# Agzs/BlockMaze

Measured on AMD Instinct MI355X. Metric: Groth16 proofs/sec (send circuit, alt_bn128), higher is better.
Workload: dtype u32 limbs (254-bit Fq/Fr Montgomery; all MSM accumulations, the H query's weighted bucket sum and the transforms' tiles on nine 29-bit limbs)

## Files before the change

### blockmaze_amd/csrc/capi_engine.cpp

```cpp
#include <cstring>
#include <memory>
#include <mutex>
#include <string>
#include <vector>
#include "../../include/zkgpu.h"
#include "gpu.hpp"

namespace zk {
void probe_field(int field, int op, const uint8_t *a, const uint8_t *b, uint8_t *out, size_t n);
void probe_fq2(int op, const uint8_t *a, const uint8_t *b, uint8_t *out, size_t n);
void probe_group(int group, int op, const uint8_t *a, const uint8_t *b, uint8_t *out, size_t n);
}
using namespace zk;
using namespace zk::host;

static thread_local std::string g_err;
void zkgpu_set_error(const std::string &s) { g_err = s; }
std::mutex g_gpu_mutex;

template <class Fn> static int guarded(Fn fn) {
  try { if (!gpu_available()) { g_err = "no HIP device visible; libzkgpu has no CPU fallback"; return ZKGPU_ERR_NO_DEVICE; }
        std::lock_guard<std::mutex> lk(g_gpu_mutex); return fn(); }
  catch (const std::exception &e) { g_err = e.what(); return ZKGPU_ERR_RUNTIME; }
  catch (...) { g_err = "unknown error"; return ZKGPU_ERR_RUNTIME; }
// ... 92 lines not shown
  while (rs < small) rs <<= 1;
  size_t m = (small == rs) ? min_size : big + rs;
  return lg <= 28 ? m : 0;
}
int zkgpu_domain_transform(size_t min_size, int op, uint8_t *data) { return guarded([&] { Domain d(min_size); size_t m = d.m(); DevBuf<Fe32> buf(m);
    buf.upload((const Fe32 *)data, m); fr_to_mont_dev(buf.get(), m);
  switch (op) {
    case 0: d.fft(buf.get(), 1, m);
    break;
    case 1: d.ifft(buf.get(), 1, m);
    break;
    case 2: d.coset_fft(buf.get(), 1, m);
    break;
    case 3: d.icoset_fft(buf.get(), 1, m);
    break;
    default: g_err = "op";
    return ZKGPU_ERR_ARG;
  }
  fr_from_mont_dev(buf.get(), m); buf.download((Fe32 *)data, m); return ZKGPU_OK; }); }

struct zkgpu_r1cs { R1csHost host; std::unique_ptr<R1csDev> dev; std::unique_ptr<Domain> dom; };
zkgpu_r1cs *zkgpu_r1cs_create(size_t n_inputs, size_t n_vars, size_t n_cons, const uint32_t *const rowptr[3], const uint32_t *const col[3],
    const uint8_t *const coeff[3]) {
  zkgpu_r1cs *out = nullptr;
  guarded([&] { std::unique_ptr<zkgpu_r1cs> h(new zkgpu_r1cs); h->host.n_inputs = n_inputs; h->host.n_vars = n_vars; h->host.n_cons = n_cons;
    for (int m = 0; m < 3; m++) {
      size_t nnz = rowptr[m][n_cons];
      h->host.rowptr[m].assign(rowptr[m], rowptr[m] + n_cons + 1);
      h->host.col[m].assign(col[m], col[m] + nnz);
      h->host.coeff[m].resize(nnz);
// ... 21 lines not shown
```

### blockmaze_amd/csrc/gen_field29.py

```python
#!/usr/bin/env python3
Q = 21888242871839275222246405745257275088696311157297823662689037894645226208583
B = 29; M = (1 << B) - 1; NL = 9; RP = 1 << (B * NL)
def limbs29(x, n=NL): return [(x >> (B * i)) & M for i in range(n - 1)] + [x >> (B * (n - 1))]
def adjusted(c):
    l = limbs29(c * Q); lo = 3 * (1 << B) + 64
    for i in range(NL - 1):
        n = 3 if l[i] + 3 * (1 << B) >= lo else 4
        l[i] += n << B; l[i + 1] -= n
        assert lo <= l[i] < 4 << B, (c, i, l[i])
    assert l[NL - 1] > 0 and sum(v << (B * i) for i, v in enumerate(l)) == c * Q
    return l
def adjusted_light(c):
    l = limbs29(c * Q); lo = (1 << B) + 64
    for i in range(NL - 1):
        n = 1 if l[i] + (1 << B) >= lo else 2
        l[i] += n << B; l[i + 1] -= n
        assert lo <= l[i] < lo + (1 << B), (c, i, l[i])
    assert l[NL - 1] > 0 and sum(v << (B * i) for i, v in enumerate(l)) == c * Q
    return l
INV = (-pow(Q, -1, 1 << B)) % (1 << B)
P29 = limbs29(Q); ONE29 = limbs29(RP % Q); RCONV = limbs29((1 << 256) % Q)
KS = {c: adjusted(c) for c in (2, 4, 6, 12, 18)}

RATIO = RP / Q
# ... 304 lines not shown
        for i in range(8): f[i + 1] += f[i] >> B; f[i] &= M
        assert (V % Q == 0) == any(f == limbs29(k * Q) for k in range(5))
lin_check()
BOUNDS_G2 = check_bounds_g2()
prm = ["// GENERATED by gen_field29.py - do not edit.  Constants of Fq on nine 29-bit limbs, for host and device code (verify_sched.hpp).", "#pragma once", "#include <cstdint>", "namespace zk { namespace p29 {"]
def carr(name, v, comment=""): prm.append("constexpr uint32_t %s[9] = {%s};%s" % (name, ", ".join("0x%xu" % x for x in v), ("   // " + comment) if comment else ""))
prm.append("constexpr uint32_t MASK = 0x%xu, INV = 0x%xu, MU = 0x%xu, MU_SHIFT = %d, LIN_MAX_UNITS = %d;   // MU = floor(2^53 / ((p >> 232) + 1)); a linear combination's value stays below LIN_MAX_UNITS p" % (M, INV, MU, MU_SHIFT, LIN_MAX_UNITS))
carr("P", P29, "p"); carr("K6", KS[6], "6 p, low limbs in [3 * 2^29 + 64, 4 * 2^29): K6 - x has no negative limb for x below 6 p with limbs below 3 * (2^29 + 8)"); carr("NP", NP, "2^264 - p (top limb: 32 bits)")
prm.append("constexpr uint32_t KP[5][9] = {%s};   // k p, k = 0 .. 4, exact limbs" % ", ".join("{" + ", ".join("0x%xu" % x for x in limbs29(k * Q)) + "}" for k in range(5)))
prm.append("} }")
open(__file__.replace("gen_field29.py", "field29_params.h"), "w").write("\n".join(prm) + "\n")
EMIT_BARRETT = True; FQ_LINES = gen_struct(); EMIT_BARRETT = False
R_MOD = 21888242871839275222246405745257275088548364400416034343698204186575808495617
Q_SAVE = Q; KS_SAVE = KS; Q = R_MOD; INV = (-pow(Q, -1, 1 << B)) % (1 << B); P29 = limbs29(Q); ONE29 = limbs29(RP % Q); RCONV = limbs29((1 << 256) % Q); KS = {}
FR_LINES = [l.replace("Fq29", "Fr29") for l in gen_struct()]; self_check()
open(__file__.replace("gen_field29.py", "field29_gfx950.inc"), "w").write("\n".join(HEADER + FQ_LINES + FR_LINES) + "\n")
print("bounds:", BOUNDS); print("bounds of the oct addition:", BOUNDS_OCT)
```

### blockmaze_amd/csrc/gpu.hip

```cpp
#include <hip/hip_runtime.h>
#include <cstdio>
#include <cstdlib>
#include <chrono>
#include <cstring>
#include <map>
#include <vector>
#include <algorithm>
#include <mutex>
#include <atomic>
#include <mutex>
#include "gpu_internal.hpp"
#include "ntt.cuh"
#include "ecntt.cuh"

__attribute__((constructor(101))) static void zkgpu_load_time_environment() { setenv("GPU_MAX_HW_QUEUES", "16", 0); }

namespace zk {

constexpr int MAX_LANES_PER_DEVICE = 31, MAX_LANES = 1 + 8 * 28;
static uint8_t g_lane_claimed[MAX_LANES];
static std::atomic<GpuContext *> g_lanes[MAX_LANES];
static std::atomic<int> g_lane_slot[MAX_LANES];
static std::mutex g_lane_mutex;
static thread_local int t_lane = 0;
// ... 227 lines not shown
  if (bytes % 16 || (reinterpret_cast<uintptr_t>(dst) | reinterpret_cast<uintptr_t>(src)) % 16) { HIP_CHECK(hipMemcpyAsync(dst, src, bytes, hipMemcpyDeviceToDevice, gpu().stream)); return; }
  const size_t n16 = bytes / 16; hipLaunchKernelGGL(k_copy_words16, dim3((unsigned)std::min<size_t>(cdiv(n16, 256), 4096)), dim3(256), 0, gpu().stream, (const uint4 *)src, (uint4 *)dst, n16);
}


static size_t ceil_log2(size_t n) { size_t r = ((n & (n - 1)) == 0 ? 0 : 1); while (n > 1) { n >>= 1; r++; } return r; }
using host::HFr;
static HFr fr_root_of_unity(size_t n) {
  HFr w;
  memcpy(w.l, FR_ROOT_OF_UNITY_2_28, 32);
  for (size_t i = 28; i > ceil_log2(n); --i) w = w.sqr();
  return w;
}
static HFr fr_coset_gen() { HFr g; memcpy(g.l, FR_COSET_GEN, 32); return g; }

struct Radix2Tables {
  int logn; size_t n; DevBuf<Fe32> tw, itw, tw261, itw261;
  Radix2Tables(size_t n_, const HFr &w) : logn((int)ceil_log2(n_)), n(n_), tw(n_ / 2 ? n_ / 2 : 1), itw(n_ / 2 ? n_ / 2 : 1), tw261(n_ / 2 ? n_ / 2 : 1),
      itw261(n_ / 2 ? n_ / 2 : 1) {
    std::vector<Fe32> a(n / 2 ? n / 2 : 1), b(a.size()), a5(a.size()), b5(a.size()); HFr wi = w.inv(), x = HFr::one(), y = HFr::one();
    auto times32 = [](HFr v) {
      for (int i = 0; i < 5; i++) v = v + v;
      return v;
    };
    for (size_t j = 0; j < std::max<size_t>(n / 2, 1); j++) {
      memcpy(&a[j], x.l, 32);
      memcpy(&b[j], y.l, 32);
      HFr x5 = times32(x), y5 = times32(y);
      memcpy(&a5[j], x5.l, 32);
      memcpy(&b5[j], y5.l, 32);
      x = x * w;
      y = y * wi;
    }
    tw.upload(a.data(), a.size()); itw.upload(b.data(), b.size()); tw261.upload(a5.data(), a5.size()); itw261.upload(b5.data(), b5.size());
  }
};
static std::vector<Fe32> geometric_table(size_t n, const HFr &first, const HFr &ratio) {
  std::vector<Fe32> t(n);
  HFr x = first;
  for (size_t i = 0; i < n; i++) {
    memcpy(&t[i], x.l, 32);
    x = x * ratio;
  }
  return t;
}

static int ntt_pref_log_c() {
  static const int v = [] {
    const char *e = getenv("ZK_NTT_LOGC");
    int x = e ? atoi(e) : 1;
    return x < 0 ? 0 : x > 3 ? 3 : x; }(); return v; }
static Fe32 fe261(HFr v) {
  for (int i = 0; i < 5; i++) v = v + v;
  Fe32 o;
  memcpy(&o, v.l, 32);
  return o;
}
struct NttCall { Fe32 *data, *scratch; const Fe32 *tw, *tw261; int logn; const Fe32 *pre_scale, *pre261; Fe32 scale261; const Fe32 *post_scale;
    size_t stride, scratch_stride; const Fe32 *out261 = nullptr; };
static int ntt_prio_bits() { static const int v = (int)(zk_prio_bits(ZKP_NTT) >> 24) << 8; return v; }
static int ntt_radix_log() {
  static const int rl = [] {
    const char *e = getenv("ZK_NTT_RADIX_LOG");
    int x = e ? atoi(e) : 2;
    return x < 1 ? 1 : x > 3 ? 3 : x;
  }();
  return rl;
}
static bool ntt_two_pass(int logn) { return logn > NTT_TILE_LOG && logn <= 2 * NTT_TILE_LOG; }
static unsigned ntt_threads_for(int logN, int logC) {
  int g = logN + logC - ntt_radix_log();
  return 1u << (g < 6 ? 6 : g > 8 ? 8 : g);
}
static size_t ntt_lds_for(int logN, int logC) {
  size_t e = (size_t)1 << (logN + logC);
  return sizeof(Fr29) * (e + (e >> 4) + 1) + (sizeof(Fr29) << logN) / 2;
}
static void ntt_raise_lds() {
  static std::atomic<uint64_t> cols_done{0}, rows_done{0};
  zk_raise_dynamic_lds((const void *)k_ntt_cols, 128 * 1024, cols_done); zk_raise_dynamic_lds((const void *)k_ntt_rows, 128 * 1024, rows_done);
}
static void ntt_two_pass_launch(const NttCall *calls, int n_calls, int batch) {
  hipStream_t s = gpu().stream;
  ntt_raise_lds();
  NttJob cj[2], rj[2];
  memset(cj, 0, sizeof cj);
  memset(rj, 0, sizeof rj);
  unsigned tc = 64, tr = 64;
  size_t lc = 0, lr = 0;
  for (int k = 0; k < n_calls; k++) {
    const NttCall &c = calls[k];
    const int l1 = c.logn / 2, l2 = c.logn - l1, c1 = std::min(ntt_pref_log_c(), std::min(NTT_TILE_LOG - l1, l2)), c2 = std::min(ntt_pref_log_c(),
        std::min(NTT_TILE_LOG - l2, l1));
    Fr sc; memcpy(&sc, &c.scale261, 32);
    cj[k] = NttJob{(const Fr *)c.data, (Fr *)c.scratch, (const Fr *)c.pre261, (const Fr *)c.tw261, sc, c.logn, l1, c1, 1u << (l2 - c1), c.stride,
        c.scratch_stride, nullptr};
    rj[k] = NttJob{(const Fr *)c.scratch, (Fr *)c.data, (const Fr *)c.post_scale, (const Fr *)c.tw261, sc, c.logn, l1, c2, 1u << (l1 - c2), c.scratch_stride,
        c.stride, (const Fr *)c.out261};
    tc = std::max(tc, ntt_threads_for(l1, c1));
    tr = std::max(tr, ntt_threads_for(l2, c2));
    lc = std::max(lc, ntt_lds_for(l1, c1));
    lr = std::max(lr, ntt_lds_for(l2, c2));
  }
  hipLaunchKernelGGL(k_ntt_cols, dim3(cj[0].tiles + cj[1].tiles, batch), dim3(tc), lc, s, cj[0], cj[1], ntt_radix_log() | ntt_prio_bits());
  hipLaunchKernelGGL(k_ntt_rows, dim3(rj[0].tiles + rj[1].tiles, batch), dim3(tr), lr, s, rj[0], rj[1], ntt_radix_log() | ntt_prio_bits());
}
static void radix2_transform(const NttCall &c, int batch) {
  hipStream_t s = gpu().stream;
  size_t n = (size_t)1 << c.logn;
  Fe32 *data = c.data, *scratch = c.scratch;
  const int logn = c.logn;
  const size_t stride = c.stride, scratch_stride = c.scratch_stride;
  if (logn <= NTT_TILE_LOG) {
    if (c.post_scale) throw GpuError("ntt: post scale on a single-pass transform");
    ntt_raise_lds();
    Fr sc;
    memcpy(&sc, &c.scale261, 32);
    if (c.out261) throw GpuError("ntt: output factors on a single-pass transform");
    NttJob j{(const Fr *)data, (Fr *)data, (const Fr *)c.pre261, (const Fr *)c.tw261, sc, logn, logn, 0, 1u, stride, stride, nullptr}, none;
    memset(&none, 0, sizeof none);
// ... 150 lines not shown
size_t Domain::m() const { return impl->m; }
bool Domain::is_step() const { return impl->step; }

static void mul_table(Fe32 *a, const Fe32 *t, size_t n, int batch, size_t stride) {
  hipLaunchKernelGGL(k_fr_mul_table, dim3(cdiv(n, 256), batch), dim3(256), 0, gpu().stream, (Fr *)a, (const Fr *)t, (uint32_t)n, stride);
}

void Domain::fft(Fe32 *data, int batch, size_t stride) { fft_with_factors(data, batch, stride, nullptr); }
void Domain::fft_with_factors(Fe32 *data, int batch, size_t stride, const Fe32 *cf) {
  Stage st("ntt.forward");
  Impl &d = *impl;
  if (batch > 3) throw GpuError("domain: batch > 3");
  if (!d.step && cf) throw GpuError("domain: factors on a basic domain go through coset_fft");
  if (!d.step) {
    radix2_transform(NttCall{data, d.scratch.get(), d.big->tw.get(), d.big->tw261.get(), d.big->logn, nullptr, nullptr, d.one261, nullptr, stride,
        d.scratch_stride}, batch);
    return;
  }
  hipStream_t s = gpu().stream; Fe32 *dbuf = d.scratch.get(), *tmp = d.scratch.get() + 3 * d.B;
  hipLaunchKernelGGL(k_step_fwd_pre, dim3(cdiv(d.B, 256), batch), dim3(256), 0, s, (Fr *)data, (Fr *)dbuf, (const Fr *)d.wpow.get(), (const Fr *)cf,
      (uint32_t)d.B, zk_with_prio(d.S, ZKP_STEP), stride);
  hipLaunchKernelGGL(k_step_fold, dim3(cdiv(d.S, 256), batch), dim3(256), 0, s, (const Fr *)dbuf, (Fr *)data, (uint32_t)d.B, zk_with_prio(d.S, ZKP_STEP), stride);
  radix2_transform_pair(NttCall{data, tmp, d.big->tw.get(), d.big->tw261.get(), d.big->logn, nullptr, nullptr, d.one261, nullptr, stride, d.B},
      NttCall{data + d.B, dbuf, d.small->tw.get(), d.small->tw261.get(), d.small->logn, nullptr, nullptr, d.one261, nullptr, stride, d.B}, batch);
}
void Domain::ifft(Fe32 *data, int batch, size_t stride) {
  Stage st("ntt.inverse"); Impl &d = *impl; if (batch > 3) throw GpuError("domain: batch > 3");
  if (!d.step) {
    radix2_transform(NttCall{data, d.scratch.get(), d.big->itw.get(), d.big->itw261.get(), d.big->logn, d.scale_big.get(), nullptr, d.inv_big261, nullptr,
        stride, d.scratch_stride}, batch);
    return;
  }
  hipStream_t s = gpu().stream; Fe32 *tmp = d.scratch.get() + 3 * d.B;
  radix2_transform_pair(NttCall{data, tmp, d.big->itw.get(), d.big->itw261.get(), d.big->logn, d.scale_big.get(), nullptr, d.inv_big261, nullptr, stride, d.B},
      NttCall{data + d.B, d.scratch.get(), d.small->itw.get(), d.small->itw261.get(), d.small->logn, d.scale_small.get(), nullptr, d.inv_small261, nullptr,
      stride, d.B}, batch);
  Fr half; memcpy(&half, d.half.l, 32);
  hipLaunchKernelGGL(k_step_inv_post, dim3(cdiv(d.S, 256), batch), dim3(256), 0, s, (Fr *)data, (const Fr *)d.wpow.get(), (const Fr *)d.winvpow.get(), half,
      (uint32_t)d.B, zk_with_prio(d.S, ZKP_STEP), stride);
}
void Domain::ifft_then_coset_fft(Fe32 *data, int batch, size_t stride) {
  Impl &d = *impl;
  if (batch > 3) throw GpuError("domain: batch > 3");
  if (!d.step) {
    if (!d.t->inv_coset261.get()) { ifft(data, batch, stride); coset_fft(data, batch, stride); return; }
    { Stage st("ntt.inverse");
      radix2_transform(NttCall{data, d.scratch.get(), d.big->itw.get(), d.big->itw261.get(), d.big->logn, nullptr, nullptr, d.inv_big261, nullptr, stride,
          d.scratch_stride, d.t->inv_coset261.get()}, batch); }
    { Stage st("ntt.forward");
      radix2_transform(NttCall{data, d.scratch.get(), d.big->tw.get(), d.big->tw261.get(), d.big->logn, nullptr, nullptr, d.one261, nullptr, stride,
          d.scratch_stride}, batch); }
    return;
  }
  hipStream_t s = gpu().stream;
  Fe32 *dbuf = d.scratch.get(), *tmp = d.scratch.get() + 3 * d.B;
  Fr half;
  memcpy(&half, d.half.l, 32);
  { Stage st("ntt.inverse");
    radix2_transform_pair(NttCall{data, tmp, d.big->itw.get(), d.big->itw261.get(), d.big->logn, d.scale_big.get(), nullptr, d.inv_big261, nullptr, stride,
        d.B}, NttCall{data + d.B, dbuf, d.small->itw.get(), d.small->itw261.get(), d.small->logn, d.scale_small.get(), nullptr, d.inv_small261, nullptr,
        stride, d.B}, batch);
    hipLaunchKernelGGL(k_step_inv_fwd, dim3(cdiv(d.S, 256), batch), dim3(256), 0, s, (Fr *)data, (const Fr *)d.wpow.get(), (const Fr *)d.winvpow.get(), half,
        (const Fr *)d.coset_fwd.get(), (uint32_t)d.B, zk_with_prio(d.S, ZKP_STEP), stride);
  }
  { Stage st("ntt.forward");
    radix2_transform_pair(NttCall{data, tmp, d.big->tw.get(), d.big->tw261.get(), d.big->logn, nullptr, nullptr, d.one261, nullptr, stride, d.B},
        NttCall{data + d.B, dbuf, d.small->tw.get(), d.small->tw261.get(), d.small->logn, nullptr, nullptr, d.one261, nullptr, stride, d.B}, batch);
  }
}
void Domain::coset_fft(Fe32 *data, int batch, size_t stride) {
  Impl &d = *impl; if (batch > 3) throw GpuError("domain: batch > 3");
  if (!d.step) {
    Stage st("ntt.forward");
    radix2_transform(NttCall{data, d.scratch.get(), d.big->tw.get(), d.big->tw261.get(), d.big->logn, d.coset_fwd.get(), d.coset_fwd261.get(), d.one261,
        nullptr, stride, d.scratch_stride}, batch);
    return;
  }
  fft_with_factors(data, batch, stride, d.coset_fwd.get());
}
void Domain::icoset_fft(Fe32 *data, int batch, size_t stride) {
  Impl &d = *impl;
  if (!d.step) { Stage st("ntt.inverse");
    if (d.big->logn <= NTT_TILE_LOG) {
      radix2_transform(NttCall{data, d.scratch.get(), d.big->itw.get(), d.big->itw261.get(), d.big->logn, nullptr, nullptr, d.one261, nullptr, stride,
          d.scratch_stride}, batch);
      mul_table(data, d.coset_inv.get(), d.m, batch, stride);
    }
    else radix2_transform(NttCall{data, d.scratch.get(), d.big->itw.get(), d.big->itw261.get(), d.big->logn, nullptr, nullptr, d.one261, d.coset_inv.get(),
        stride, d.scratch_stride}, batch);
    return; }
  ifft(data, batch, stride); mul_table(data, d.coset_inv.get(), d.m, batch, stride);
}
bool Domain::supports_h_lagrange() const { return true; }
void Domain::h_query_to_coset_lagrange(const G1AffineRaw *h, size_t n_in, G1AffineRaw *out) {
  Impl &d = *impl; if (n_in > d.m) throw GpuError("domain: h_query_to_coset_lagrange"); hipStream_t s = gpu().stream; const size_t m = d.m;
  DevBuf<G1AffineRaw> din(n_in ? n_in : 1), dout(m);
  DevBuf<uint8_t> data(m * sizeof(XYZZ<Fq>));
  if (n_in) din.upload(h, n_in);
  XYZZ<Fq> *X = (XYZZ<Fq> *)data.get();
  auto idft = [&](XYZZ<Fq> *part, const Radix2Tables &t, Affine<Fq> *o) {
    for (int st = t.logn; st >= 1; st--) hipLaunchKernelGGL(k_ecntt_stage, dim3(cdiv(t.n / 2, 64)), dim3(64), 0, s, part, (const Fr *)t.itw.get(), t.logn, st);
    hipLaunchKernelGGL(k_ecntt_finish, dim3(cdiv(t.n, 64)), dim3(64), 0, s, (const XYZZ<Fq> *)part, t.logn, o); };
  hipLaunchKernelGGL(k_ecntt_prescale, dim3(cdiv(m, 64)), dim3(64), 0, s, (const Affine<Fq> *)din.get(), (uint32_t)n_in, (const Fr *)d.coset_inv.get(),
      (uint32_t)m, X);
// ... 210 lines not shown
```

### blockmaze_amd/csrc/ntt.cuh

```cuda
#pragma once
#include <hip/hip_runtime.h>
#include "field.cuh"
#include "field29.cuh"

namespace zk {

constexpr int NTT_LOCAL_LOG = 10;
constexpr int NTT_LOCAL_THREADS = 512;

__device__ __forceinline__ uint32_t bitrev32(uint32_t x, int bits) { return __brev(x) >> (32 - bits); }

__global__ void k_ntt_bitrev_scale(const Fr *__restrict__ in, Fr *__restrict__ out, const Fr *__restrict__ scale, int logn, size_t stride_in,
    size_t stride_out) {
  uint32_t i = blockIdx.x * blockDim.x + threadIdx.x, n = 1u << logn; if (i >= n) return;
  const Fr *src = in + blockIdx.y * stride_in; Fr *dst = out + blockIdx.y * stride_out; uint32_t r = bitrev32(i, logn);
  Fr v = src[r]; if (scale) v = v * scale[r]; dst[i] = v;
}

__global__ void __launch_bounds__(NTT_LOCAL_THREADS) k_ntt_local(Fr *__restrict__ data, const Fr *__restrict__ tw, int logn, int L, size_t stride) {
  extern __shared__ uint32_t lds_raw[]; Fr *tile = reinterpret_cast<Fr *>(lds_raw);
  const uint32_t T = 1u << L, half_n = 1u << (logn - 1); Fr *d = data + blockIdx.y * stride + (size_t)blockIdx.x * T;
  for (uint32_t i = threadIdx.x; i < T; i += blockDim.x) tile[i] = d[i];
  __syncthreads();
  for (int s = 1; s <= L; s++) {
// ... 39 lines not shown
#pragma unroll
      for (int q = 0; q < (1 << R); q++) if (!(q & hx)) {
        const uint32_t blk = (base + ((uint32_t)q << sh)) >> st; Fr29 u = x[q], v = x[q + hx];
        if (bits) v = Fr29::mul(v, twl[(__brev(blk) >> (32 - bits)) << (st - 1)]);
        const Fr29 sum = Fr29::add_raw(u, v), dif = Fr29::sub_product(u, v);
        const bool carry_now = (t & 1) == 1 || t == R - 1;
        x[q] = carry_now ? sum.norm() : sum;
        x[q + hx] = carry_now ? dif.norm() : dif;
      }
    }
#pragma unroll
    for (int q = 0; q < (1 << R); q++) tile[ntt_pad(((base + ((uint32_t)q << sh)) << logC) + c)] = x[q];
  }
  __syncthreads();
}
__device__ __forceinline__ void ntt29_lds_transform(Fr29 *tile, Fr29 *twl, int logN, int logC, const Fr *__restrict__ tw261, uint32_t tws, int radix_log) {
  for (uint32_t j = threadIdx.x; j < (1u << logN) / 2; j += blockDim.x) twl[j] = ntt29_from_words(tw261[j * tws]);
  __syncthreads();
  int s = logN;
  if (radix_log >= 3) for (; s >= 3; s -= 3) ntt29_lds_pass<3>(tile, twl, logN, logC, s);
  if (radix_log >= 2) for (; s >= 2; s -= 2) ntt29_lds_pass<2>(tile, twl, logN, logC, s);
  for (; s >= 1; s -= 1) ntt29_lds_pass<1>(tile, twl, logN, logC, s);
}
struct NttJob {
  const Fr *src;
  Fr *dst;
  const Fr *factor;
  const Fr *tw261;
  Fr scale261;
  int logn, log_n1, logC;
  uint32_t tiles;
  size_t stride_in, stride_out;
  const Fr *out261;
};
__global__ void __launch_bounds__(NTT_TILE_THREADS) k_ntt_cols(NttJob ja, NttJob jb, int radix_log) {
  { const int prio = radix_log >> 8; radix_log &= 0xff; if (prio == 1) __builtin_amdgcn_s_setprio(1); else if (prio == 2) __builtin_amdgcn_s_setprio(2); else if (prio == 3) __builtin_amdgcn_s_setprio(3); }
  extern __shared__ uint32_t lds_raw[]; Fr29 *tile = reinterpret_cast<Fr29 *>(lds_raw);
  const bool second = blockIdx.x >= ja.tiles; const NttJob j = second ? jb : ja;
  const uint32_t bid = blockIdx.x - (second ? ja.tiles : 0u);
  const int logn = j.logn, log_n1 = j.log_n1, logC = j.logC; const Fr *__restrict__ tw261 = j.tw261; const Fr *__restrict__ pre261 = j.factor;
  const uint32_t n_tiles = j.tiles, tile_no = n_tiles >= 8 && n_tiles % 8 == 0 ? (bid % 8) * (n_tiles / 8) + bid / 8 : bid;
  const int log_n2 = logn - log_n1;
  const uint32_t n2 = 1u << log_n2, C = 1u << logC, c0 = tile_no << logC, elems = (1u << log_n1) << logC, half_n = logn ? 1u << (logn - 1) : 1u;
  const Fr *s = j.src + blockIdx.y * j.stride_in; Fr *d = j.dst + blockIdx.y * j.stride_out;
  for (uint32_t w = threadIdx.x; w < elems; w += blockDim.x) {
    uint32_t g = ((w >> logC) << log_n2) + c0 + (w & (C - 1));
    Fr29 v = ntt29_from_words(s[g]);
    if (pre261) v = Fr29::mul(ntt29_from_words(pre261[g]), v);
    tile[ntt_pad(w)] = v;
  }
  __syncthreads();
  ntt29_lds_transform(tile, tile + ntt_pad(elems), log_n1, logC, tw261, n2, radix_log);
  for (uint32_t w = threadIdx.x; w < elems; w += blockDim.x) {
    uint32_t k1 = w >> logC, c = w & (C - 1), i2 = c0 + c, p = log_n1 ? bitrev32(k1, log_n1) : 0; const Fr29 v = tile[ntt_pad((p << logC) + c)];
    const uint32_t e = i2 * k1;
    Fr29 t = ntt29_from_words(log_n2 ? tw261[e < half_n ? e : e - half_n] : j.scale261);
    if (e >= half_n) t = Fr29::neg_product(t);
    d[(k1 << log_n2) + i2] = ntt29_to_words(Fr29::mul(t, v));
  }
}
__global__ void __launch_bounds__(NTT_TILE_THREADS) k_ntt_rows(NttJob ja, NttJob jb, int radix_log) {
  { const int prio = radix_log >> 8; radix_log &= 0xff; if (prio == 1) __builtin_amdgcn_s_setprio(1); else if (prio == 2) __builtin_amdgcn_s_setprio(2); else if (prio == 3) __builtin_amdgcn_s_setprio(3); }
  extern __shared__ uint32_t lds_raw[]; Fr29 *tile = reinterpret_cast<Fr29 *>(lds_raw);
  const bool second = blockIdx.x >= ja.tiles; const NttJob &j = second ? jb : ja; const uint32_t bid = blockIdx.x - (second ? ja.tiles : 0u);
  const int logn = j.logn, log_n1 = j.log_n1, logC = j.logC;
  const Fr *__restrict__ tw261 = j.tw261;
  const Fr *__restrict__ post = j.factor;
  const Fr *__restrict__ out261 = j.out261;
  const int log_n2 = logn - log_n1; const uint32_t n2 = 1u << log_n2, C = 1u << logC, r0 = bid << logC, elems = n2 << logC;
  const Fr *s = j.src + blockIdx.y * j.stride_in; Fr *d = j.dst + blockIdx.y * j.stride_out;
  for (uint32_t w = threadIdx.x; w < elems; w += blockDim.x) {
    uint32_t c = w >> log_n2, i2 = w & (n2 - 1);
    tile[ntt_pad((i2 << logC) + c)] = ntt29_from_words(s[((size_t)(r0 + c) << log_n2) + i2]);
  }
  __syncthreads();
  ntt29_lds_transform(tile, tile + ntt_pad(elems), log_n2, logC, tw261, 1u << log_n1, radix_log);
  const Fr29 one = ntt29_from_words(j.scale261);
  for (uint32_t w = threadIdx.x; w < elems; w += blockDim.x) {
    uint32_t k2 = w >> logC, c = w & (C - 1), p = bitrev32(k2, log_n2), o = (k2 << log_n1) + r0 + c;
    const Fr29 f = out261 ? ntt29_from_words(out261[o]) : one;
    Fr v = ntt29_to_words(Fr29::mul(f, tile[ntt_pad((p << logC) + c)]));
    if (post) v = v * post[o];
    d[o] = v;
  }
}

__global__ void k_fr_mul_table(Fr *__restrict__ a, const Fr *__restrict__ table, uint32_t n, size_t stride) {
  uint32_t i = blockIdx.x * blockDim.x + threadIdx.x; if (i >= n) return; Fr *d = a + blockIdx.y * stride; d[i] = d[i] * table[i];
}
__global__ void k_qap_pointwise(Fr *__restrict__ a, const Fr *__restrict__ b, const Fr *__restrict__ c, const Fr *__restrict__ zinv, int zinv_is_table,
    uint32_t n) {
  uint32_t i = blockIdx.x * blockDim.x + threadIdx.x;
  if (i >= n) return;
  Fr t = a[i] * b[i];
  if (c) t = t - c[i];
  a[i] = t * zinv[zinv_is_table ? i : 0];
}
__global__ void k_fr_to_mont(Fr *__restrict__ a, uint32_t n) { uint32_t i = blockIdx.x * blockDim.x + threadIdx.x; if (i < n) a[i] = a[i].to_mont(); }
// ... 263 lines not shown
```

### blockmaze_amd/engine.py

```python
import ctypes, os
import numpy as np

_HERE = os.path.dirname(os.path.abspath(__file__))
LIB_PATH = os.path.join(_HERE, "libzkgpu.so")
if os.environ.get("ZKGPU_LIB"): LIB_PATH = os.environ["ZKGPU_LIB"]

class ZkGpuError(RuntimeError):
    pass

_lib = None
def lib():
    global _lib
    if _lib is None:
        if not os.path.exists(LIB_PATH):
            raise ZkGpuError("%s not built: run `python -c 'import __graft_entry__ as g; g.build()'` (hipcc, gfx950)" % LIB_PATH)
        L = ctypes.CDLL(LIB_PATH)
        L.zkgpu_last_error.restype = ctypes.c_char_p; L.zkgpu_version.restype = ctypes.c_char_p
        L.zkgpu_domain_size.restype = ctypes.c_size_t; L.zkgpu_domain_size.argtypes = [ctypes.c_size_t]
        L.zkgpu_msm_create.restype = ctypes.c_void_p; L.zkgpu_r1cs_create.restype = ctypes.c_void_p
        _lib = L
    return _lib

def _check(rc):
    if rc != 0:
# ... 34 lines not shown
        self.h = lib().zkgpu_msm_create(group, _bytes(points), ctypes.c_size_t(self.n), int(window_bits), int(filter_ones))
        if not self.h: raise ZkGpuError(lib().zkgpu_last_error().decode())
    def set_scalars(self, scalars):
        scalars = np.ascontiguousarray(scalars, dtype=np.uint64); _check(lib().zkgpu_msm_set_scalars(ctypes.c_void_p(self.h), _bytes(scalars), ctypes.c_size_t(scalars.size // 4)))
    def run(self):
        out = np.zeros(8 if self.group == 1 else 16, dtype=np.uint64); _check(lib().zkgpu_msm_run(ctypes.c_void_p(self.h), _bytes(out))); return out
    def close(self):
        if self.h: lib().zkgpu_msm_destroy(ctypes.c_void_p(self.h)); self.h = None
    def __del__(self):
        try: self.close()
        except Exception: pass

def domain_size(min_size): return int(lib().zkgpu_domain_size(min_size))
def domain_transform(min_size, op, data):
    data = np.ascontiguousarray(data, dtype=np.uint64).copy()
    _check(lib().zkgpu_domain_transform(ctypes.c_size_t(min_size), {"fft": 0, "ifft": 1, "cosetfft": 2, "icosetfft": 3}[op], _bytes(data))); return data

class R1cs:
    def __init__(self, n_inputs, n_vars, n_cons, rowptr, col, coeff):
        self.n_inputs, self.n_vars, self.n_cons = n_inputs, n_vars, n_cons
        self._keep = [[np.ascontiguousarray(x, dtype=np.uint32) for x in rowptr], [np.ascontiguousarray(x, dtype=np.uint32) for x in col], [np.ascontiguousarray(x, dtype=np.uint64) for x in coeff]]
        P32 = ctypes.POINTER(ctypes.c_uint32); P8 = ctypes.POINTER(ctypes.c_uint8)
        rp = (P32 * 3)(*[x.ctypes.data_as(P32) for x in self._keep[0]]); cl = (P32 * 3)(*[x.ctypes.data_as(P32) for x in self._keep[1]]); co = (P8 * 3)(*[x.ctypes.data_as(P8) for x in self._keep[2]])
        self.h = lib().zkgpu_r1cs_create(ctypes.c_size_t(n_inputs), ctypes.c_size_t(n_vars), ctypes.c_size_t(n_cons), rp, cl, co)
        if not self.h: raise ZkGpuError(lib().zkgpu_last_error().decode())
        self.m = domain_size(n_cons + n_inputs + 1)
    def witness_map(self, z):
        z = np.ascontiguousarray(z, dtype=np.uint64); H = np.zeros((self.m + 1, 4), dtype=np.uint64)
        _check(lib().zkgpu_witness_map(ctypes.c_void_p(self.h), _bytes(z), _bytes(H))); return H
    def close(self):
        if self.h: lib().zkgpu_r1cs_destroy(ctypes.c_void_p(self.h)); self.h = None
# ... 376 lines not shown
```

Before: 1339.

## Fuse inverse-NTT rows with forward-NTT columns and precompute 29-bit twiddle tables

For power-of-two domains in the two-pass range, the ifft-then-coset-fft sequence drops from four tile kernels to three. A new kernel runs the inverse rows pass, applies the coset factor, then runs the forward columns pass in DIT order on the same LDS tile, which removes one global round trip. Twiddles are also precomputed in 29-bit limb form on the host and copied straight into LDS instead of being converted on every launch. The cost is extra twiddle memory, a new DIT pass with looser lazy-reduction bounds (checked in the generator script), and an env switch to turn the fusion off.

```diff
diff --git a/blockmaze_amd/csrc/capi_engine.cpp b/blockmaze_amd/csrc/capi_engine.cpp
--- a/blockmaze_amd/csrc/capi_engine.cpp
+++ b/blockmaze_amd/csrc/capi_engine.cpp
@@ -130,6 +130,8 @@
     break;
     case 3: d.icoset_fft(buf.get(), 1, m);
     break;
+    case 4: d.ifft_then_coset_fft(buf.get(), 1, m);
+    break;
     default: g_err = "op";
     return ZKGPU_ERR_ARG;
   }
diff --git a/blockmaze_amd/csrc/gen_field29.py b/blockmaze_amd/csrc/gen_field29.py
--- a/blockmaze_amd/csrc/gen_field29.py
+++ b/blockmaze_amd/csrc/gen_field29.py
@@ -342,5 +342,16 @@
 R_MOD = 21888242871839275222246405745257275088548364400416034343698204186575808495617
 Q_SAVE = Q; KS_SAVE = KS; Q = R_MOD; INV = (-pow(Q, -1, 1 << B)) % (1 << B); P29 = limbs29(Q); ONE29 = limbs29(RP % Q); RCONV = limbs29((1 << 256) % Q); KS = {}
 FR_LINES = [l.replace("Fq29", "Fr29") for l in gen_struct()]; self_check()
+def check_bounds_ntt_fused():
+    ratio = RP / Q; v = 2.0; kl2 = adjusted_light(2)
+    for stage in range(11):
+        t = v / ratio + 1.0
+        assert t < 2.0 and kl2[NL - 1] >= int(t * Q) >> (B * (NL - 1)), (stage, t)
+        v += max(t, 2.0)
+    assert v <= 2 + 11 * 2.2 and int(v * Q) + 1 < RP
+    assert (int(v * Q) >> (B * (NL - 1))) + 4 < (1 << 29), v
+    assert v / ratio + 1.0 < 2.0 and 2 * Q < 1 << 256
+    return v
+BOUNDS_NTT_FUSED = check_bounds_ntt_fused()
 open(__file__.replace("gen_field29.py", "field29_gfx950.inc"), "w").write("\n".join(HEADER + FQ_LINES + FR_LINES) + "\n")
 print("bounds:", BOUNDS); print("bounds of the oct addition:", BOUNDS_OCT)
diff --git a/blockmaze_amd/csrc/gpu.hip b/blockmaze_amd/csrc/gpu.hip
--- a/blockmaze_amd/csrc/gpu.hip
+++ b/blockmaze_amd/csrc/gpu.hip
@@ -265,8 +265,20 @@
 }
 static HFr fr_coset_gen() { HFr g; memcpy(g.l, FR_COSET_GEN, 32); return g; }
 
+static void fr29_limbs(const Fe32 &v, uint32_t *l) {
+  for (int i = 0; i < 9; i++) {
+    const int bit = 29 * i, j = bit >> 5, sh = bit & 31;
+    uint64_t x = v.l[j] >> sh;
+    if (j + 1 < 8) x |= (uint64_t)v.l[j + 1] << (32 - sh);
+    l[i] = i < 8 ? (uint32_t)x & 0x1fffffffu : (uint32_t)x;
+  }
+}
+struct NttTwc { const uint32_t *lo = nullptr, *hi = nullptr; };
 struct Radix2Tables {
   int logn; size_t n; DevBuf<Fe32> tw, itw, tw261, itw261;
+  DevBuf<uint32_t> twc[2][2];
+  NttTwc twc_fwd() const { return NttTwc{twc[0][0].get(), twc[0][1].get()}; }
+  NttTwc twc_inv() const { return NttTwc{twc[1][0].get(), twc[1][1].get()}; }
   Radix2Tables(size_t n_, const HFr &w) : logn((int)ceil_log2(n_)), n(n_), tw(n_ / 2 ? n_ / 2 : 1), itw(n_ / 2 ? n_ / 2 : 1), tw261(n_ / 2 ? n_ / 2 : 1),
       itw261(n_ / 2 ? n_ / 2 : 1) {
     std::vector<Fe32> a(n / 2 ? n / 2 : 1), b(a.size()), a5(a.size()), b5(a.size()); HFr wi = w.inv(), x = HFr::one(), y = HFr::one();
@@ -284,6 +296,13 @@
       y = y * wi;
     }
     tw.upload(a.data(), a.size()); itw.upload(b.data(), b.size()); tw261.upload(a5.data(), a5.size()); itw261.upload(b5.data(), b5.size());
+    if (logn > NTT_TILE_LOG && logn <= 2 * NTT_TILE_LOG)
+      for (int dir = 0; dir < 2; dir++) for (int hi = 0; hi < 2; hi++) {
+        const int logN = hi ? logn - logn / 2 : logn / 2; const size_t half = ((size_t)1 << logN) / 2, step = n >> logN;
+        const std::vector<Fe32> &src = dir ? b5 : a5; std::vector<uint32_t> limbs(9 * half);
+        for (size_t j = 0; j < half; j++) fr29_limbs(src[j * step], &limbs[9 * j]);
+        twc[dir][hi] = DevBuf<uint32_t>(limbs.size()); twc[dir][hi].upload(limbs.data(), limbs.size());
+      }
   }
 };
 static std::vector<Fe32> geometric_table(size_t n, const HFr &first, const HFr &ratio) {
@@ -308,7 +327,7 @@
   return o;
 }
 struct NttCall { Fe32 *data, *scratch; const Fe32 *tw, *tw261; int logn; const Fe32 *pre_scale, *pre261; Fe32 scale261; const Fe32 *post_scale;
-    size_t stride, scratch_stride; const Fe32 *out261 = nullptr; };
+    size_t stride, scratch_stride; const Fe32 *out261 = nullptr; NttTwc twc = {}; };
 static int ntt_prio_bits() { static const int v = (int)(zk_prio_bits(ZKP_NTT) >> 24) << 8; return v; }
 static int ntt_radix_log() {
   static const int rl = [] {
@@ -328,9 +347,11 @@
   return sizeof(Fr29) * (e + (e >> 4) + 1) + (sizeof(Fr29) << logN) / 2;
 }
 static void ntt_raise_lds() {
-  static std::atomic<uint64_t> cols_done{0}, rows_done{0};
+  static std::atomic<uint64_t> cols_done{0}, rows_done{0}, fused_done{0};
   zk_raise_dynamic_lds((const void *)k_ntt_cols, 128 * 1024, cols_done); zk_raise_dynamic_lds((const void *)k_ntt_rows, 128 * 1024, rows_done);
-}
+  zk_raise_dynamic_lds((const void *)k_ntt_rows_cols, 128 * 1024, fused_done);
+}
+static bool ntt_fused() { static const bool on = [] { const char *e = getenv("ZK_NTT_FUSED"); return !(e && *e == '0'); }(); return on; }
 static void ntt_two_pass_launch(const NttCall *calls, int n_calls, int batch) {
   hipStream_t s = gpu().stream;
   ntt_raise_lds();
@@ -345,9 +366,9 @@
         std::min(NTT_TILE_LOG - l2, l1));
     Fr sc; memcpy(&sc, &c.scale261, 32);
     cj[k] = NttJob{(const Fr *)c.data, (Fr *)c.scratch, (const Fr *)c.pre261, (const Fr *)c.tw261, sc, c.logn, l1, c1, 1u << (l2 - c1), c.stride,
-        c.scratch_stride, nullptr};
+        c.scratch_stride, nullptr, (const Fr29 *)c.twc.lo};
     rj[k] = NttJob{(const Fr *)c.scratch, (Fr *)c.data, (const Fr *)c.post_scale, (const Fr *)c.tw261, sc, c.logn, l1, c2, 1u << (l1 - c2), c.scratch_stride,
-        c.stride, (const Fr *)c.out261};
+        c.stride, (const Fr *)c.out261, (const Fr29 *)c.twc.hi};
     tc = std::max(tc, ntt_threads_for(l1, c1));
     tr = std::max(tr, ntt_threads_for(l2, c2));
     lc = std::max(lc, ntt_lds_for(l1, c1));
@@ -355,6 +376,28 @@
   }
   hipLaunchKernelGGL(k_ntt_cols, dim3(cj[0].tiles + cj[1].tiles, batch), dim3(tc), lc, s, cj[0], cj[1], ntt_radix_log() | ntt_prio_bits());
   hipLaunchKernelGGL(k_ntt_rows, dim3(rj[0].tiles + rj[1].tiles, batch), dim3(tr), lr, s, rj[0], rj[1], ntt_radix_log() | ntt_prio_bits());
+}
+static void ntt_fused_launch(const NttCall &inv, const NttCall &fwd, int batch, int launch) {
+  hipStream_t s = gpu().stream;
+  ntt_raise_lds();
+  const int logn = inv.logn, l1 = logn / 2, l2 = logn - l1, c1 = std::min(ntt_pref_log_c(), std::min(NTT_TILE_LOG - l1, l2)), c2 = std::min(ntt_pref_log_c(),
+      std::min(NTT_TILE_LOG - l2, l1));
+  if (!ntt_two_pass(logn) || fwd.logn != logn || fwd.data != inv.data || fwd.stride != inv.stride || !inv.out261 || !inv.twc.lo || !fwd.twc.lo)
+    throw GpuError("ntt: fused launch outside its range");
+  Fr si, sf; memcpy(&si, &inv.scale261, 32); memcpy(&sf, &fwd.scale261, 32);
+  NttJob none; memset(&none, 0, sizeof none);
+  const NttJob icol{(const Fr *)inv.data, (Fr *)inv.data, nullptr, (const Fr *)inv.tw261, si, logn, l1, c1, 1u << (l2 - c1), inv.stride, inv.stride, nullptr,
+      (const Fr29 *)inv.twc.lo};
+  const NttJob irow{(const Fr *)inv.data, nullptr, nullptr, (const Fr *)inv.tw261, si, logn, l1, c2, 1u << (l1 - c2), inv.stride, 0, (const Fr *)inv.out261,
+      (const Fr29 *)inv.twc.hi};
+  const NttJob fcol{nullptr, (Fr *)inv.scratch, nullptr, (const Fr *)fwd.tw261, sf, logn, l2, c2, 1u << (l1 - c2), 0, inv.scratch_stride, nullptr,
+      (const Fr29 *)fwd.twc.hi};
+  const NttJob frow{(const Fr *)inv.scratch, (Fr *)fwd.data, (const Fr *)fwd.post_scale, (const Fr *)fwd.tw261, sf, logn, l2, c1, 1u << (l2 - c1),
+      inv.scratch_stride, fwd.stride, nullptr, (const Fr29 *)fwd.twc.lo};
+  const int rl = ntt_radix_log() | ntt_prio_bits();
+  if (launch == 0) hipLaunchKernelGGL(k_ntt_cols, dim3(icol.tiles, batch), dim3(ntt_threads_for(l1, c1)), ntt_lds_for(l1, c1), s, icol, none, rl);
+  else if (launch == 1) hipLaunchKernelGGL(k_ntt_rows_cols, dim3(irow.tiles, batch), dim3(ntt_threads_for(l2, c2)), ntt_lds_for(l2, c2), s, irow, fcol, rl);
+  else hipLaunchKernelGGL(k_ntt_rows, dim3(frow.tiles, batch), dim3(ntt_threads_for(l1, c1)), ntt_lds_for(l1, c1), s, frow, none, rl);
 }
 static void radix2_transform(const NttCall &c, int batch) {
   hipStream_t s = gpu().stream;
@@ -535,27 +578,27 @@
   if (!d.step && cf) throw GpuError("domain: factors on a basic domain go through coset_fft");
   if (!d.step) {
     radix2_transform(NttCall{data, d.scratch.get(), d.big->tw.get(), d.big->tw261.get(), d.big->logn, nullptr, nullptr, d.one261, nullptr, stride,
-        d.scratch_stride}, batch);
+        d.scratch_stride, nullptr, d.big->twc_fwd()}, batch);
     return;
   }
   hipStream_t s = gpu().stream; Fe32 *dbuf = d.scratch.get(), *tmp = d.scratch.get() + 3 * d.B;
   hipLaunchKernelGGL(k_step_fwd_pre, dim3(cdiv(d.B, 256), batch), dim3(256), 0, s, (Fr *)data, (Fr *)dbuf, (const Fr *)d.wpow.get(), (const Fr *)cf,
       (uint32_t)d.B, zk_with_prio(d.S, ZKP_STEP), stride);
   hipLaunchKernelGGL(k_step_fold, dim3(cdiv(d.S, 256), batch), dim3(256), 0, s, (const Fr *)dbuf, (Fr *)data, (uint32_t)d.B, zk_with_prio(d.S, ZKP_STEP), stride);
-  radix2_transform_pair(NttCall{data, tmp, d.big->tw.get(), d.big->tw261.get(), d.big->logn, nullptr, nullptr, d.one261, nullptr, stride, d.B},
-      NttCall{data + d.B, dbuf, d.small->tw.get(), d.small->tw261.get(), d.small->logn, nullptr, nullptr, d.one261, nullptr, stride, d.B}, batch);
+  radix2_transform_pair(NttCall{data, tmp, d.big->tw.get(), d.big->tw261.get(), d.big->logn, nullptr, nullptr, d.one261, nullptr, stride, d.B, nullptr, d.big->twc_fwd()},
+      NttCall{data + d.B, dbuf, d.small->tw.get(), d.small->tw261.get(), d.small->logn, nullptr, nullptr, d.one261, nullptr, stride, d.B, nullptr, d.small->twc_fwd()}, batch);
 }
 void Domain::ifft(Fe32 *data, int batch, size_t stride) {
   Stage st("ntt.inverse"); Impl &d = *impl; if (batch > 3) throw GpuError("domain: batch > 3");
   if (!d.step) {
     radix2_transform(NttCall{data, d.scratch.get(), d.big->itw.get(), d.big->itw261.get(), d.big->logn, d.scale_big.get(), nullptr, d.inv_big261, nullptr,
-        stride, d.scratch_stride}, batch);
+        stride, d.scratch_stride, nullptr, d.big->twc_inv()}, batch);
     return;
   }
   hipStream_t s = gpu().stream; Fe32 *tmp = d.scratch.get() + 3 * d.B;
-  radix2_transform_pair(NttCall{data, tmp, d.big->itw.get(), d.big->itw261.get(), d.big->logn, d.scale_big.get(), nullptr, d.inv_big261, nullptr, stride, d.B},
+  radix2_transform_pair(NttCall{data, tmp, d.big->itw.get(), d.big->itw261.get(), d.big->logn, d.scale_big.get(), nullptr, d.inv_big261, nullptr, stride, d.B, nullptr, d.big->twc_inv()},
       NttCall{data + d.B, d.scratch.get(), d.small->itw.get(), d.small->itw261.get(), d.small->logn, d.scale_small.get(), nullptr, d.inv_small261, nullptr,
-      stride, d.B}, batch);
+      stride, d.B, nullptr, d.small->twc_inv()}, batch);
   Fr half; memcpy(&half, d.half.l, 32);
   hipLaunchKernelGGL(k_step_inv_post, dim3(cdiv(d.S, 256), batch), dim3(256), 0, s, (Fr *)data, (const Fr *)d.wpow.get(), (const Fr *)d.winvpow.get(), half,
       (uint32_t)d.B, zk_with_prio(d.S, ZKP_STEP), stride);
@@ -565,12 +608,22 @@
   if (batch > 3) throw GpuError("domain: batch > 3");
   if (!d.step) {
     if (!d.t->inv_coset261.get()) { ifft(data, batch, stride); coset_fft(data, batch, stride); return; }
+    if (ntt_fused()) {
+      const NttCall inv{data, d.scratch.get(), d.big->itw.get(), d.big->itw261.get(), d.big->logn, nullptr, nullptr, d.inv_big261, nullptr, stride,
+          d.scratch_stride, d.t->inv_coset261.get(), d.big->twc_inv()},
+          fwd{data, d.scratch.get(), d.big->tw.get(), d.big->tw261.get(), d.big->logn, nullptr, nullptr, d.one261, nullptr, stride, d.scratch_stride, nullptr,
+          d.big->twc_fwd()};
+      { Stage st("ntt.inverse"); ntt_fused_launch(inv, fwd, batch, 0); }
+      { Stage st("ntt.middle"); ntt_fused_launch(inv, fwd, batch, 1); }
+      { Stage st("ntt.forward"); ntt_fused_launch(inv, fwd, batch, 2); }
+      return;
+    }
     { Stage st("ntt.inverse");
       radix2_transform(NttCall{data, d.scratch.get(), d.big->itw.get(), d.big->itw261.get(), d.big->logn, nullptr, nullptr, d.inv_big261, nullptr, stride,
-          d.scratch_stride, d.t->inv_coset261.get()}, batch); }
+          d.scratch_stride, d.t->inv_coset261.get(), d.big->twc_inv()}, batch); }
     { Stage st("ntt.forward");
       radix2_transform(NttCall{data, d.scratch.get(), d.big->tw.get(), d.big->tw261.get(), d.big->logn, nullptr, nullptr, d.one261, nullptr, stride,
-          d.scratch_stride}, batch); }
+          d.scratch_stride, nullptr, d.big->twc_fwd()}, batch); }
     return;
   }
   hipStream_t s = gpu().stream;
@@ -579,14 +632,14 @@
   memcpy(&half, d.half.l, 32);
   { Stage st("ntt.inverse");
     radix2_transform_pair(NttCall{data, tmp, d.big->itw.get(), d.big->itw261.get(), d.big->logn, d.scale_big.get(), nullptr, d.inv_big261, nullptr, stride,
-        d.B}, NttCall{data + d.B, dbuf, d.small->itw.get(), d.small->itw261.get(), d.small->logn, d.scale_small.get(), nullptr, d.inv_small261, nullptr,
-        stride, d.B}, batch);
+        d.B, nullptr, d.big->twc_inv()}, NttCall{data + d.B, dbuf, d.small->itw.get(), d.small->itw261.get(), d.small->logn, d.scale_small.get(), nullptr, d.inv_small261, nullptr,
+        stride, d.B, nullptr, d.small->twc_inv()}, batch);
     hipLaunchKernelGGL(k_step_inv_fwd, dim3(cdiv(d.S, 256), batch), dim3(256), 0, s, (Fr *)data, (const Fr *)d.wpow.get(), (const Fr *)d.winvpow.get(), half,
         (const Fr *)d.coset_fwd.get(), (uint32_t)d.B, zk_with_prio(d.S, ZKP_STEP), stride);
   }
   { Stage st("ntt.forward");
-    radix2_transform_pair(NttCall{data, tmp, d.big->tw.get(), d.big->tw261.get(), d.big->logn, nullptr, nullptr, d.one261, nullptr, stride, d.B},
-        NttCall{data + d.B, dbuf, d.small->tw.get(), d.small->tw261.get(), d.small->logn, nullptr, nullptr, d.one261, nullptr, stride, d.B}, batch);
+    radix2_transform_pair(NttCall{data, tmp, d.big->tw.get(), d.big->tw261.get(), d.big->logn, nullptr, nullptr, d.one261, nullptr, stride, d.B, nullptr, d.big->twc_fwd()},
+        NttCall{data + d.B, dbuf, d.small->tw.get(), d.small->tw261.get(), d.small->logn, nullptr, nullptr, d.one261, nullptr, stride, d.B, nullptr, d.small->twc_fwd()}, batch);
   }
 }
 void Domain::coset_fft(Fe32 *data, int batch, size_t stride) {
@@ -594,7 +647,7 @@
   if (!d.step) {
     Stage st("ntt.forward");
     radix2_transform(NttCall{data, d.scratch.get(), d.big->tw.get(), d.big->tw261.get(), d.big->logn, d.coset_fwd.get(), d.coset_fwd261.get(), d.one261,
-        nullptr, stride, d.scratch_stride}, batch);
+        nullptr, stride, d.scratch_stride, nullptr, d.big->twc_fwd()}, batch);
     return;
   }
   fft_with_factors(data, batch, stride, d.coset_fwd.get());
@@ -604,11 +657,11 @@
   if (!d.step) { Stage st("ntt.inverse");
     if (d.big->logn <= NTT_TILE_LOG) {
       radix2_transform(NttCall{data, d.scratch.get(), d.big->itw.get(), d.big->itw261.get(), d.big->logn, nullptr, nullptr, d.one261, nullptr, stride,
-          d.scratch_stride}, batch);
+          d.scratch_stride, nullptr, d.big->twc_inv()}, batch);
       mul_table(data, d.coset_inv.get(), d.m, batch, stride);
     }
     else radix2_transform(NttCall{data, d.scratch.get(), d.big->itw.get(), d.big->itw261.get(), d.big->logn, nullptr, nullptr, d.one261, d.coset_inv.get(),
-        stride, d.scratch_stride}, batch);
+        stride, d.scratch_stride, nullptr, d.big->twc_inv()}, batch);
     return; }
   ifft(data, batch, stride); mul_table(data, d.coset_inv.get(), d.m, batch, stride);
 }
diff --git a/blockmaze_amd/csrc/ntt.cuh b/blockmaze_amd/csrc/ntt.cuh
--- a/blockmaze_amd/csrc/ntt.cuh
+++ b/blockmaze_amd/csrc/ntt.cuh
@@ -77,13 +77,50 @@
   }
   __syncthreads();
 }
-__device__ __forceinline__ void ntt29_lds_transform(Fr29 *tile, Fr29 *twl, int logN, int logC, const Fr *__restrict__ tw261, uint32_t tws, int radix_log) {
-  for (uint32_t j = threadIdx.x; j < (1u << logN) / 2; j += blockDim.x) twl[j] = ntt29_from_words(tw261[j * tws]);
-  __syncthreads();
+template <int R> __device__ __forceinline__ void ntt29_lds_pass_dit(Fr29 *tile, const Fr29 *twl, int logN, int logC, int s) {
+  const uint32_t groups = (1u << (logN - R)) << logC, cmask = (1u << logC) - 1; const int sh = s - 1;
+  for (uint32_t w = threadIdx.x; w < groups; w += blockDim.x) {
+    const uint32_t g = w >> logC, c = w & cmask, base = ((g >> sh) << (sh + R)) | (g & ((1u << sh) - 1)); Fr29 x[1 << R];
+#pragma unroll
+    for (int q = 0; q < (1 << R); q++) x[q] = tile[ntt_pad(((base + ((uint32_t)q << sh)) << logC) + c)];
+#pragma unroll
+    for (int t = 0; t < R; t++) {
+      const int st = s + t, hx = 1 << t;
+#pragma unroll
+      for (int q = 0; q < (1 << R); q++) if (!(q & hx)) {
+        const uint32_t j = (base + ((uint32_t)q << sh)) & ((1u << (st - 1)) - 1); Fr29 u = x[q], v = x[q + hx];
+        if (st > 1) v = Fr29::mul(v, twl[j << (logN - st)]);
+        const Fr29 sum = Fr29::add_raw(u, v), dif = Fr29::sub_product(u, v);
+        const bool carry_now = (t & 1) == 1 || t == R - 1;
+        x[q] = carry_now ? sum.norm() : sum;
+        x[q + hx] = carry_now ? dif.norm() : dif;
+      }
+    }
+#pragma unroll
+    for (int q = 0; q < (1 << R); q++) tile[ntt_pad(((base + ((uint32_t)q << sh)) << logC) + c)] = x[q];
+  }
+  __syncthreads();
+}
+__device__ __forceinline__ void ntt29_load_twiddles(Fr29 *twl, int logN, const Fr *__restrict__ tw261, uint32_t tws, const Fr29 *__restrict__ twc) {
+  const uint32_t half = (1u << logN) / 2;
+  if (twc) { const uint32_t *src = reinterpret_cast<const uint32_t *>(twc); uint32_t *dst = reinterpret_cast<uint32_t *>(twl);
+    for (uint32_t i = threadIdx.x; i < half * 9; i += blockDim.x) dst[i] = src[i]; }
+  else for (uint32_t j = threadIdx.x; j < half; j += blockDim.x) twl[j] = ntt29_from_words(tw261[j * tws]);
+  __syncthreads();
+}
+__device__ __forceinline__ void ntt29_lds_transform(Fr29 *tile, Fr29 *twl, int logN, int logC, const Fr *__restrict__ tw261, uint32_t tws, int radix_log,
+    const Fr29 *__restrict__ twc) {
+  ntt29_load_twiddles(twl, logN, tw261, tws, twc);
   int s = logN;
   if (radix_log >= 3) for (; s >= 3; s -= 3) ntt29_lds_pass<3>(tile, twl, logN, logC, s);
   if (radix_log >= 2) for (; s >= 2; s -= 2) ntt29_lds_pass<2>(tile, twl, logN, logC, s);
   for (; s >= 1; s -= 1) ntt29_lds_pass<1>(tile, twl, logN, logC, s);
+}
+__device__ __forceinline__ void ntt29_lds_transform_dit(Fr29 *tile, const Fr29 *twl, int logN, int logC, int radix_log) {
+  int s = 1;
+  if (radix_log >= 3) for (; s + 2 <= logN; s += 3) ntt29_lds_pass_dit<3>(tile, twl, logN, logC, s);
+  if (radix_log >= 2) for (; s + 1 <= logN; s += 2) ntt29_lds_pass_dit<2>(tile, twl, logN, logC, s);
+  for (; s <= logN; s += 1) ntt29_lds_pass_dit<1>(tile, twl, logN, logC, s);
 }
 struct NttJob {
   const Fr *src;
@@ -95,6 +132,7 @@
   uint32_t tiles;
   size_t stride_in, stride_out;
   const Fr *out261;
+  const Fr29 *twc;
 };
 __global__ void __launch_bounds__(NTT_TILE_THREADS) k_ntt_cols(NttJob ja, NttJob jb, int radix_log) {
   { const int prio = radix_log >> 8; radix_log &= 0xff; if (prio == 1) __builtin_amdgcn_s_setprio(1); else if (prio == 2) __builtin_amdgcn_s_setprio(2); else if (prio == 3) __builtin_amdgcn_s_setprio(3); }
@@ -113,7 +151,7 @@
     tile[ntt_pad(w)] = v;
   }
   __syncthreads();
-  ntt29_lds_transform(tile, tile + ntt_pad(elems), log_n1, logC, tw261, n2, radix_log);
+  ntt29_lds_transform(tile, tile + ntt_pad(elems), log_n1, logC, tw261, n2, radix_log, j.twc);
   for (uint32_t w = threadIdx.x; w < elems; w += blockDim.x) {
     uint32_t k1 = w >> logC, c = w & (C - 1), i2 = c0 + c, p = log_n1 ? bitrev32(k1, log_n1) : 0; const Fr29 v = tile[ntt_pad((p << logC) + c)];
     const uint32_t e = i2 * k1;
@@ -137,7 +175,7 @@
     tile[ntt_pad((i2 << logC) + c)] = ntt29_from_words(s[((size_t)(r0 + c) << log_n2) + i2]);
   }
   __syncthreads();
-  ntt29_lds_transform(tile, tile + ntt_pad(elems), log_n2, logC, tw261, 1u << log_n1, radix_log);
+  ntt29_lds_transform(tile, tile + ntt_pad(elems), log_n2, logC, tw261, 1u << log_n1, radix_log, j.twc);
   const Fr29 one = ntt29_from_words(j.scale261);
   for (uint32_t w = threadIdx.x; w < elems; w += blockDim.x) {
     uint32_t k2 = w >> logC, c = w & (C - 1), p = bitrev32(k2, log_n2), o = (k2 << log_n1) + r0 + c;
@@ -145,6 +183,34 @@
     Fr v = ntt29_to_words(Fr29::mul(f, tile[ntt_pad((p << logC) + c)]));
     if (post) v = v * post[o];
     d[o] = v;
+  }
+}
+__global__ void __launch_bounds__(NTT_TILE_THREADS) k_ntt_rows_cols(NttJob ji, NttJob jf, int radix_log) {
+  { const int prio = radix_log >> 8; radix_log &= 0xff; if (prio == 1) __builtin_amdgcn_s_setprio(1); else if (prio == 2) __builtin_amdgcn_s_setprio(2); else if (prio == 3) __builtin_amdgcn_s_setprio(3); }
+  extern __shared__ uint32_t lds_raw[]; Fr29 *tile = reinterpret_cast<Fr29 *>(lds_raw);
+  const int logn = ji.logn, log_n1 = ji.log_n1, logC = ji.logC, log_n2 = logn - log_n1;
+  const uint32_t n_tiles = ji.tiles, bid = blockIdx.x, tile_no = n_tiles >= 8 && n_tiles % 8 == 0 ? (bid % 8) * (n_tiles / 8) + bid / 8 : bid;
+  const uint32_t n2 = 1u << log_n2, C = 1u << logC, r0 = tile_no << logC, elems = n2 << logC, half_n = 1u << (logn - 1);
+  const Fr *s = ji.src + blockIdx.y * ji.stride_in; Fr *d = jf.dst + blockIdx.y * jf.stride_out;
+  const Fr *__restrict__ out261 = ji.out261; const Fr *__restrict__ ftw261 = jf.tw261;
+  Fr29 *twl = tile + ntt_pad(elems);
+  for (uint32_t w = threadIdx.x; w < elems; w += blockDim.x) {
+    uint32_t c = w >> log_n2, i2 = w & (n2 - 1);
+    tile[ntt_pad((i2 << logC) + c)] = ntt29_from_words(s[((size_t)(r0 + c) << log_n2) + i2]);
+  }
+  __syncthreads();
+  ntt29_lds_transform(tile, twl, log_n2, logC, ji.tw261, 1u << log_n1, radix_log, ji.twc);
+  for (uint32_t w = threadIdx.x; w < elems; w += blockDim.x) {
+    const uint32_t k2 = w >> logC, c = w & (C - 1), at = ntt_pad((bitrev32(k2, log_n2) << logC) + c);
+    tile[at] = Fr29::mul(ntt29_from_words(out261[(k2 << log_n1) + r0 + c]), tile[at]);
+  }
+  ntt29_load_twiddles(twl, log_n2, ftw261, 1u << log_n1, jf.twc);
+  ntt29_lds_transform_dit(tile, twl, log_n2, logC, radix_log);
+  for (uint32_t w = threadIdx.x; w < elems; w += blockDim.x) {
+    const uint32_t k1 = w >> logC, i2 = r0 + (w & (C - 1)), e = i2 * k1;
+    Fr29 t = ntt29_from_words(ftw261[e < half_n ? e : e - half_n]);
+    if (e >= half_n) t = Fr29::neg_product(t);
+    d[((size_t)k1 << log_n1) + i2] = ntt29_to_words(Fr29::mul(t, tile[ntt_pad(w)]));
   }
 }
 
diff --git a/blockmaze_amd/engine.py b/blockmaze_amd/engine.py
--- a/blockmaze_amd/engine.py
+++ b/blockmaze_amd/engine.py
@@ -72,7 +72,7 @@
 def domain_size(min_size): return int(lib().zkgpu_domain_size(min_size))
 def domain_transform(min_size, op, data):
     data = np.ascontiguousarray(data, dtype=np.uint64).copy()
-    _check(lib().zkgpu_domain_transform(ctypes.c_size_t(min_size), {"fft": 0, "ifft": 1, "cosetfft": 2, "icosetfft": 3}[op], _bytes(data))); return data
+    _check(lib().zkgpu_domain_transform(ctypes.c_size_t(min_size), {"fft": 0, "ifft": 1, "cosetfft": 2, "icosetfft": 3, "ifft_cosetfft": 4}[op], _bytes(data))); return data
 
 class R1cs:
     def __init__(self, n_inputs, n_vars, n_cons, rowptr, col, coeff):
```

Result: no change. 1331 (-0.6%).
